# neu-vi/Superpoints_Registration

Hardware: AMD Instinct MI355X
Metric: point-cloud pairs/sec (16 384 pts/cloud) (higher is better)
Workload: dtype f32 (matrix products: range-scaled split-f16x2 MFMA, f32 accumulate; attention weights below 2^-5 of their row sum carried in one f16 plane); 1 GPU; synthetic 16384-pt pairs, full KPConv backbone + superpoint attn + Sinkhorn-SVD pose (3dmatch config, BASELINE configs[1]); streams_per_gpu=1, points_per_cloud=16384, generator=box, point_order=reference, upsample_indices=True, cross_step_overlap=True, streams_inside_a_forward=3: main path, pyramid searches, ResNet shortcut branches

## Files before the change

superpoints_registration_amd/csrc/kpconv.hip:

```cpp
#include "lds_dma.h"
#include "spr_common.h"
#include "split_mma.h"

namespace spr {
namespace {

constexpr int kKP = 15;

__global__ __launch_bounds__(256) void k_rowflag(const float* __restrict__ x, const float* __restrict__ s_xyz,
                                                 int ns, int cin, unsigned char* __restrict__ flag,
                                                 float4* __restrict__ sxf, int* __restrict__ tile_ctr) {
  const int wid = (blockIdx.x * blockDim.x + threadIdx.x) >> 6;
  const int lane = threadIdx.x & 63;
  const int c4 = cin >> 2;
  if (blockIdx.x == 0 && threadIdx.x == 0) {
    sxf[ns] = make_float4(-1.0e17f, -1.0e17f, -1.0e17f, __int_as_float(0));
    tile_ctr[0] = 0;
  }
  if ((cin & 3) == 0 && c4 <= 64 && (c4 & (c4 - 1)) == 0) {
    constexpr int kRfSteps = 4;
    const int rpl = 64 / c4;
    const int sub = lane / c4, chunk = lane % c4;
    const int row0 = wid * rpl * kRfSteps + sub;
    float4 v[kRfSteps];
// ... 428 lines not shown
  const int qv = lane & 15, g = lane >> 4;
  const int q0 = blockIdx.x * 64 + wave * 16;
  const int q = q0 + qv;
  float mx = 0.f;
  if (q0 < nq) {
    float b[4];
    stem_load_group(S, q0, nq, qv, g, b);
    const int cloud = find_segment(cu, nb, min(q, nq - 1));
    for (int o0 = 0; o0 < cout; o0 += 16) {
      f32x4 acc = {0.f, 0.f, 0.f, 0.f};
#pragma unroll
      for (int s = 0; s < 4; ++s) {
        const float av = 4 * s + g < n_kp ? W[(size_t)(4 * s + g) * cout + o0 + qv] : 0.f;
        acc = __builtin_amdgcn_mfma_f32_16x16x4f32(av, b[s], acc, 0, 0, 0);
      }
      if (q < nq) {
        const float4 m = *reinterpret_cast<const float4*>(mean + (size_t)cloud * cout + o0 + 4 * g);
        const float4 r = *reinterpret_cast<const float4*>(rstd + (size_t)cloud * cout + o0 + 4 * g);
        float4 w;
        w.x = (acc[0] - m.x) * r.x;
        w.y = (acc[1] - m.y) * r.y;
        w.z = (acc[2] - m.z) * r.z;
        w.w = (acc[3] - m.w) * r.w;
        w.x = w.x >= 0.f ? w.x : w.x * slope;
        w.y = w.y >= 0.f ? w.y : w.y * slope;
        w.z = w.z >= 0.f ? w.z : w.z * slope;
        w.w = w.w >= 0.f ? w.w : w.w * slope;
        *reinterpret_cast<float4*>(out + (size_t)q * cout + o0 + 4 * g) = w;
        mx = fmaxf(mx, fmaxf(fmaxf(fabsf(w.x), fabsf(w.y)), fmaxf(fabsf(w.z), fabsf(w.w))));
      }
    }
  }
  if (out_range != nullptr) publish_range(mx, out_range, nslots);
}

__global__ __launch_bounds__(256) void k_w_prep(const float* __restrict__ W, int cin, int cout, int cc,
                                                const float* __restrict__ w_parts, int n_wparts,
                                                _Float16* __restrict__ Wh, _Float16* __restrict__ Wl) {
  __shared__ float sh[17];
  const float sb = pow2f(pow2_exp_for(block_absmax(w_parts, sh, n_wparts)));
  const int total = kKP * cin * cout;
  const int i = blockIdx.x * blockDim.x + threadIdx.x;
  if (i >= total) return;
  const int KS = kKP * cc / 32, NT = cout / 16;
  const int e = i & 7, lane = (i >> 3) & 63;
  int r = i >> 9;
  const int ks = r % KS;
  r /= KS;
  const int nt = r % NT, chunk = r / NT;
  const int p16 = lane & 15, j4 = lane >> 4;
  const int kk = 32 * ks + 8 * j4 + e;
  const int p = kk / cc, c = chunk * cc + kk % cc;
  const float w = W[((size_t)p * cin + c) * cout + 16 * nt + p16] * sb;
  const _Float16 h = (_Float16)w;
  Wh[i] = h;
  Wl[i] = (_Float16)(w - (float)h);
}

#define KP_TILE_COUNTS(W) W(0) W(2) W(4) W(6) W(8) W(12) W(16)
SPR_DEFINE_WAIT_VM_ANY(wait_vm_tile, KP_TILE_COUNTS)

template <int N> struct VecF;
template <> struct VecF<2> { typedef f32x2 type; };
template <> struct VecF<4> { typedef f32x4 type; };
template <int N> struct VecH;
template <> struct VecH<2> { typedef f16x2 type; };
template <> struct VecH<4> { typedef f16x4 type; };

template <int NTC>
struct KpItem {
  int idx[4];
  float4 sp[4];
  float b[4][NTC];
  float qx, qy, qz;
};

template <int CC, int TQ, int NTW, int NW, int SK, int P1W>
__global__ __launch_bounds__(64 * P1W) void k_kpconv_mfma(
    const float* __restrict__ q_xyz, int nq, const float* __restrict__ s_xyz, int ns,
    const int* __restrict__ nbr, int nbr_stride, int kmax, int rows_sorted,
    const float* __restrict__ x, int cin, const _Float16* __restrict__ Wh,
    const _Float16* __restrict__ Wl, int cout, const float* __restrict__ kpts, float inv_extent,
    const float4* __restrict__ sxf, const float* __restrict__ x_parts,
    const float* __restrict__ w_parts, int n_xparts, int n_wparts, float* __restrict__ out) {
  constexpr int NTC = CC / 16;
  constexpr int MT = TQ / 16;
  constexpr int KW = kKP * CC;
  constexpr int SH = KW + 16;
  constexpr int QPW = TQ / P1W;
  constexpr int NTHR = 64 * P1W;
  static_assert(P1W >= NW && TQ % P1W == 0, "phase-1 waves");
  extern __shared__ __align__(16) unsigned char lds_raw[];
  _Float16* wfh = (_Float16*)lds_raw;
  _Float16* wfl = wfh + TQ * SH;
  int* lcnt = (int*)(wfl + TQ * SH);
  int* lnit = lcnt + TQ;
  int* litem = lnit + P1W;
  const int nblk = (kmax + 15) >> 4;
  const int KP = nblk * 16;
  int* lidx = litem + P1W * QPW * nblk;

  const int tid = threadIdx.x;
  const int wave = tid >> 6, lane = tid & 63;
  const int p16 = lane & 15, j4 = lane >> 4;

  float kx = 0.f, ky = 0.f, kz = 0.f;
  if (p16 < kKP) {
    kx = kpts[3 * p16];
    ky = kpts[3 * p16 + 1];
    kz = kpts[3 * p16 + 2];
  }

  float sa, unscale;
  {
    float* shf = reinterpret_cast<float*>(lds_raw);
    const int ka = pow2_exp_for(block_absmax(x_parts, shf, n_xparts) * (float)kmax);
    const int kb = pow2_exp_for(block_absmax(w_parts, shf, n_wparts));
    __syncthreads();
    sa = pow2f(ka);
    unscale = pow2f(-ka - kb);
  }

  const int ntiles = (nq + TQ - 1) / TQ;
  for (int tile = blockIdx.x; tile < ntiles; tile += gridDim.x) {
  const int q0 = tile * TQ;

  for (int e = tid; e < TQ * KP; e += NTHR) {
    const int q = e / KP, k = e - q * KP;
    const int n = q0 + q;
    lidx[e] = (n < nq && k < kmax) ? nbr[(size_t)n * nbr_stride + k] : ns;
  }
  __syncthreads();
  {
    int n_it = 0;
    for (int qi = 0; qi < QPW; ++qi) {
      const int* row = lidx + (wave * QPW + qi) * KP;
      int nb = nblk;
      if (rows_sorted) {
        int v = 0;
        for (int k0 = 0; k0 < KP; k0 += 64) {
          const int k = k0 + lane;
          const bool ok = k < KP && row[min(k, KP - 1)] >= 0 && row[min(k, KP - 1)] < ns;
          v += __popcll(__ballot(ok));
        }
        nb = max(1, (v + 15) >> 4);
      }
      if (lane < nb) litem[wave * QPW * nblk + n_it + lane] = (qi << 8) | ((lane == nb - 1) ? 128 : 0) | lane;
      n_it += nb;
    }
    if (lane == 0) lnit[wave] = n_it;
  }
  __syncthreads();
  const int n_items = lnit[wave];
  const int* my_items = litem + wave * QPW * nblk;

  constexpr int NG = (SK == 1) ? NW / MT : NW / SK;
  constexpr int MTW = (SK == 1) ? 1 : MT;
  const int mt = (SK == 1) ? wave % MT : 0;
  const int ng = (SK == 1) ? wave / MT : wave % NG;
  const int kh = (SK == 1) ? 0 : wave / NG;
  f32x4 acc2[MTW][NTW];
#pragma unroll
  for (int m = 0; m < MTW; ++m)
#pragma unroll
    for (int t = 0; t < NTW; ++t) acc2[m][t] = (f32x4){0.f, 0.f, 0.f, 0.f};

  for (int c0 = 0; c0 < cin; c0 += CC) {
    f32x4 acc1[NTC];
#pragma unroll
    for (int t = 0; t < NTC; ++t) acc1[t] = (f32x4){0.f, 0.f, 0.f, 0.f};
    int cnt = 0;

    auto issue = [&](int it, KpItem<NTC>& I) {
      const int code = my_items[min(it, n_items - 1)];
      const int qi = code >> 8, b = code & 127;
      const int n = min(q0 + wave * QPW + qi, nq - 1);
      const int* row = lidx + (wave * QPW + qi) * KP + b * 16 + j4;
      I.qx = q_xyz[3 * (size_t)n];
      I.qy = q_xyz[3 * (size_t)n + 1];
      I.qz = q_xyz[3 * (size_t)n + 2];
#pragma unroll
      for (int s = 0; s < 4; ++s) {
        const int id_ = row[4 * s];
        I.idx[s] = id_;
        const bool ok = id_ >= 0 && id_ < ns;
        const size_t id = ok ? (size_t)id_ : 0;
        I.sp[s] = sxf[id];
        typedef typename VecF<NTC>::type vec_t;
        const vec_t xv = *reinterpret_cast<const vec_t*>(x + id * cin + c0 + NTC * p16);
#pragma unroll
        for (int t = 0; t < NTC; ++t) I.b[s][t] = xv[t];
      }
    };
    auto compute = [&](int it, const KpItem<NTC>& I) {
      if (it >= n_items) return;
      const int code = my_items[it];
#pragma unroll
      for (int s = 0; s < 4; ++s) {
        const bool ok = I.idx[s] >= 0 && I.idx[s] < ns;
        const float dx = (I.sp[s].x - I.qx) - kx, dy = (I.sp[s].y - I.qy) - ky,
                    dz = (I.sp[s].z - I.qz) - kz;
        float w = fmaxf(0.f, 1.f - __builtin_amdgcn_sqrtf(dx * dx + dy * dy + dz * dz) * inv_extent);
        if (!ok || p16 >= kKP) w = 0.f;
        cnt += (ok && c0 == 0 && p16 == 0) ? __float_as_int(I.sp[s].w) : 0;
#pragma unroll
        for (int t = 0; t < NTC; ++t) {
          acc1[t] = __builtin_amdgcn_mfma_f32_16x16x4f32(w, I.b[s][t], acc1[t], 0, 0, 0);
        }
      }
      if (code & 128) {
        const int ql = wave * QPW + (code >> 8);
#pragma unroll
        for (int r = 0; r < 4; ++r) {
          const int p = acc_row16(r, j4);
          typedef typename VecH<NTC>::type hv_t;
          hv_t hh, ll;
          if constexpr (NTC == 2) {
            unsigned int hu, lu;
            split_pk_s(acc1[0][r], acc1[1][r], sa, hu, lu);
            hh = __builtin_bit_cast(hv_t, hu);
            ll = __builtin_bit_cast(hv_t, lu);
          } else {
            static_assert(NTC == 4, "NTC is 2 or 4");
            unsigned int h0, l0, h1, l1;
            split_pk_s(acc1[0][r], acc1[1][r], sa, h0, l0);
            split_pk_s(acc1[2][r], acc1[3][r], sa, h1, l1);
            hh = __builtin_bit_cast(hv_t, (u32x2){h0, h1});
            ll = __builtin_bit_cast(hv_t, (u32x2){l0, l1});
          }
          if (p < kKP) {
            *reinterpret_cast<hv_t*>(wfh + ql * SH + p * CC + NTC * p16) = hh;
            *reinterpret_cast<hv_t*>(wfl + ql * SH + p * CC + NTC * p16) = ll;
          }
        }
#pragma unroll
        for (int t = 0; t < NTC; ++t) acc1[t] = (f32x4){0.f, 0.f, 0.f, 0.f};
        if (c0 == 0) {
          int c = cnt;
          c += __shfl_xor(c, 16, 64);
          c += __shfl_xor(c, 32, 64);
          if (lane == 0) lcnt[ql] = c;
        }
        cnt = 0;
      }
    };

    {
      KpItem<NTC> A, B;
      issue(0, A);
      for (int it = 0; it < n_items; it += 2) {
        issue(it + 1, B);
        compute(it, A);
        issue(it + 2, A);
        compute(it + 1, B);
      }
    }
    __syncthreads();
    if (wave < NW) {
      constexpr int NBATCH = KW / 32 / SK;
      const int ks0 = kh * NBATCH;
      constexpr int LPB = 2 * NTW;
      constexpr int D = (NTW <= 2) ? 5 : 3;
      static_assert(NBATCH % D == 0 && NBATCH >= 2 * D && (D - 1) * LPB <= 16, "ring shape");
      const _Float16* ah_row = wfh + (mt * 16 + p16) * SH + 8 * j4;
      const _Float16* al_row = wfl + (mt * 16 + p16) * SH + 8 * j4;
      constexpr int KS = KW / 32;
      const size_t wofs = ((size_t)(c0 / CC) * (cout / 16) + ng * NTW) * KS * 512 + lane * 8;
      f16x8 bh[D][NTW], bl[D][NTW];
      auto load_step = [&](int ks, f16x8 (&dh)[NTW], f16x8 (&dl)[NTW]) {
        const size_t gk = wofs + (size_t)(ks0 + ks) * 512;
#pragma unroll
        for (int t = 0; t < NTW; ++t) {
          const _Float16* ph = Wh + gk + (size_t)t * KS * 512;
          const _Float16* pl = Wl + gk + (size_t)t * KS * 512;
          asm volatile("global_load_dwordx4 %0, %1, off" : "=v"(dh[t]) : "v"(ph));
          asm volatile("global_load_dwordx4 %0, %1, off" : "=v"(dl[t]) : "v"(pl));
        }
      };
      auto mma_step = [&](int ks, const f16x8 (&sh)[NTW], const f16x8 (&sl)[NTW]) {
#pragma unroll
        for (int m = 0; m < MTW; ++m) {
          const f16x8 ah = *reinterpret_cast<const f16x8*>(ah_row + m * 16 * SH + 32 * (ks0 + ks));
          const f16x8 al = *reinterpret_cast<const f16x8*>(al_row + m * 16 * SH + 32 * (ks0 + ks));
#pragma unroll
          for (int t = 0; t < NTW; ++t) {
            acc2[m][t] = mma3_16(ah, al, sh[t], sl[t], acc2[m][t]);
          }
        }
      };
      wait_vm<0>();
#pragma unroll
      for (int d = 0; d < D; ++d) load_step(d, bh[d], bl[d]);
      for (int b0 = 0; b0 < NBATCH - D; b0 += D) {
#pragma unroll
        for (int d = 0; d < D; ++d) {
          wait_vm_tile((D - 1) * LPB);
          __builtin_amdgcn_sched_barrier(0);
          mma_step(b0 + d, bh[d], bl[d]);
          __builtin_amdgcn_sched_barrier(0);
          load_step(b0 + d + D, bh[d], bl[d]);
        }
      }
#pragma unroll
      for (int d = 0; d < D; ++d) {
        wait_vm_tile((D - 1 - d) * LPB);
        __builtin_amdgcn_sched_barrier(0);
        mma_step(NBATCH - D + d, bh[d], bl[d]);
      }
    }
    __syncthreads();
  }
  const bool writer = (SK == 1) ? (wave < NW) : (wave < NW && kh == 0);
  if (SK == 2) {
    float* red = reinterpret_cast<float*>(lds_raw);
    if (wave < NW && kh == 1) {
#pragma unroll
      for (int m = 0; m < MTW; ++m)
#pragma unroll
        for (int t = 0; t < NTW; ++t)
#pragma unroll
          for (int r = 0; r < 4; ++r)
            red[(((ng * MTW + m) * NTW + t) * 4 + r) * 64 + lane] = acc2[m][t][r];
    }
    __syncthreads();
    if (writer) {
#pragma unroll
      for (int m = 0; m < MTW; ++m)
#pragma unroll
        for (int t = 0; t < NTW; ++t)
#pragma unroll
          for (int r = 0; r < 4; ++r)
            acc2[m][t][r] += red[(((ng * MTW + m) * NTW + t) * 4 + r) * 64 + lane];
    }
  }
  if (writer) {
#pragma unroll
    for (int m = 0; m < MTW; ++m)
#pragma unroll
      for (int r = 0; r < 4; ++r) {
        const int ql = (mt + m) * 16 + 4 * j4 + r;
        const int n = q0 + ql;
        if (n < nq) {
          const float inv = unscale / (float)max(lcnt[ql], 1);
#pragma unroll
          for (int t = 0; t < NTW; ++t)
            out[(size_t)n * cout + (ng * NTW + t) * 16 + p16] = acc2[m][t][r] * inv;
        }
      }
  }
  __syncthreads();
  }
}

static inline size_t mfma_lds_bytes(int cc, int tq, int p1w, int kmax) {
  const int sh = kKP * cc + 16, qpw = tq / p1w, nblk = (kmax + 15) / 16;
  return 2 * sizeof(_Float16) * (size_t)tq * sh + sizeof(int) * (tq + p1w) + sizeof(int) * (size_t)p1w * qpw * nblk +
         sizeof(int) * (size_t)tq * nblk * 16;
}
constexpr size_t kMfmaLdsMax = 160 * 1024;
constexpr int kTile64TQ = 32, kTile32TQ = 64, kTileWaves = 8;

template <int CC, int TQ, int NTW, int NW, int SK, int P1W = NW>
int launch_mfma(const float* q_xyz, int nq, const float* s_xyz, int ns, const int* nbr,
                int nbr_stride, int kmax, int rows_sorted, const float* x, int cin,
                const _Float16* Wh, const _Float16* Wl, int cout, const float* kpts,
                float inv_extent, const float4* sxf, const float* x_parts, const float* w_parts, int n_xparts,
                int n_wparts, float* out, hipStream_t stream) {
  const size_t lds = mfma_lds_bytes(CC, TQ, P1W, kmax);
  auto kern = k_kpconv_mfma<CC, TQ, NTW, NW, SK, P1W>;
  ProfScope prof(stream, cin * 100000 + cout, nq);
  SPR_REQUIRE(lds <= kMfmaLdsMax, "kpconv: neighbour rows too wide for the LDS tile (kmax=%d)", kmax);
  if (lds > 64 * 1024)
    if (int rc = ensure_dyn_lds((const void*)kern, 160 * 1024)) return rc;
  const int n_cu = device_cu_count();
  const int per_cu = (int)((160 * 1024) / lds) > 0 ? (int)((160 * 1024) / lds) : 1;
  const int ntiles = cdiv(nq, TQ);
  const int grid = ntiles < n_cu * per_cu ? ntiles : n_cu * per_cu;
  hipLaunchKernelGGL(kern, dim3(grid), dim3(64 * P1W), lds, stream, q_xyz, nq, s_xyz, ns,
                     nbr, nbr_stride, kmax, rows_sorted, x, cin, Wh, Wl, cout, kpts, inv_extent,
                     sxf, x_parts, w_parts, n_xparts, n_wparts, out);
  SPR_LAUNCH_CHECK();
  return 0;
}


constexpr int kRingTQ = 16;

__global__ __launch_bounds__(256) void k_kp_tiles(const int* __restrict__ nbr, int nq, int ns, int nbr_stride,
                                                  int kmax, int rows_sorted, const int* __restrict__ order,
                                                  int ntiles, int4* __restrict__ desc, int* __restrict__ pad_word) {
  const int tile = (blockIdx.x * blockDim.x + threadIdx.x) >> 6;
  const int lane = threadIdx.x & 63;
  if (blockIdx.x == 0 && threadIdx.x == 0) pad_word[0] = ns;
  if (tile >= ntiles) return;
  int my_q = -1, my_c = 0;
  for (int r = 0; r < kRingTQ; ++r) {
    const int pos = tile * kRingTQ + r;
    int q = -1, c = 0;
    if (pos < nq) {
      q = order ? order[pos] : pos;
      if (rows_sorted) {
        int v = 0;
        for (int k0 = 0; k0 < kmax; k0 += 64) {
          const int k = k0 + lane;
          const int id = k < kmax ? nbr[(size_t)q * nbr_stride + k] : ns;
          v += __popcll(__ballot(id >= 0 && id < ns));
        }
        c = max(1, (v + 7) >> 3);
      } else {
        c = (kmax + 7) >> 3;
      }
    }
    if (lane == r) { my_q = q; my_c = c; }
  }
  int rank = 0;
  for (int j = 0; j < kRingTQ; ++j) {
    const int cj = __shfl(my_c, j, 64);
    rank += (cj > my_c || (cj == my_c && j < lane)) ? 1 : 0;
  }
  if (lane < kRingTQ) {
    int* d = reinterpret_cast<int*>(desc + (size_t)tile * 8);
    const int w = rank < 8 ? rank : 15 - rank, second = rank < 8 ? 0 : 1;
    d[w * 4 + second] = my_q;
    d[w * 4 + 2 + second] = my_c;
  }
}

#define KP_RING_COUNTS(W)                                                                                      \
  W(0) W(1) W(2) W(3) W(4) W(5) W(6) W(7) W(8) W(9) W(10) W(11) W(12) W(13) W(14) W(15) W(16) W(17) W(18) W(19) \
  W(20) W(21) W(22) W(23) W(24) W(25) W(26) W(27) W(28)
SPR_DEFINE_WAIT_VM_ANY(wait_vm_ring, KP_RING_COUNTS)

template <int CC, int COUT, int NS>
struct RingShape {
  static constexpr int NTC = CC / 16;
  static constexpr int KW = kKP * CC;
  static constexpr int SH = KW + 16;
  static constexpr int KS = KW / 32;
  static constexpr int NG = COUT / 16;
  static constexpr int SPLIT = 8 / NG;
  static constexpr int KSW = (KS + SPLIT - 1) / SPLIT;
  static constexpr int RB = CC * 4;
  static constexpr int LPR = RB / 16;
  static constexpr int RPP = 64 / LPR;
  static constexpr int PPI = 8 / RPP;
  static constexpr int DPI = PPI + 1;
  static constexpr int SLOT = 8 * RB + 128;
  static constexpr int WF_BYTES = 2 * kRingTQ * SH * 2;
  static constexpr int RED_BYTES = NG * (SPLIT - 1) * 4 * 64 * 4;
  static constexpr int RING_BYTES = 8 * NS * SLOT;
  static constexpr int SMALL_BYTES = 2 * kRingTQ * 4 * 2 + 16;
  static constexpr int MINW = (CC == 32 && COUT == 32) ? 4 : 2;
  static_assert(NG * SPLIT == 8 && NS >= 3, "shape");
  static __host__ __device__ size_t lds_bytes(int idxw) {
    return (size_t)WF_BYTES + RED_BYTES + RING_BYTES + SMALL_BYTES + (size_t)8 * 2 * 2 * idxw * 4;
  }
};

#ifdef SPR_KP_RING_PROF
constexpr int kTraceN = 160;
__device__ unsigned long long g_kp_trace[8 * kTraceN];
#define KP_STAMP(id)                                                                            \
  do {                                                                                          \
// ... 276 lines not shown
        const int ks = min(ks0 + k, KS - 1);
        const f16x8 ah = *reinterpret_cast<const f16x8*>(ah_row + 32 * ks);
        const f16x8 al = *reinterpret_cast<const f16x8*>(al_row + 32 * ks);
        acc2 = mma3_16(ah, al, bh[k], bl[k], acc2);
      }
    }
    if (sp > 0) {
#pragma unroll
      for (int r = 0; r < 4; ++r) red[((ng * (SPLIT - 1) + sp - 1) * 4 + r) * 64 + lane] = acc2[r];
    }
    KP_STAMP(6);
    asm volatile("s_waitcnt lgkmcnt(0)" ::: "memory");
    __builtin_amdgcn_s_barrier();
    KP_STAMP(7);
    if (sp == 0) {
#pragma unroll
      for (int s2 = 1; s2 < SPLIT; ++s2)
#pragma unroll
        for (int r = 0; r < 4; ++r) acc2[r] += red[((ng * (SPLIT - 1) + s2 - 1) * 4 + r) * 64 + lane];
#pragma unroll
      for (int r = 0; r < 4; ++r) {
        const int ql = acc_row16(r, j4);
        pend_n[r] = lqid[par * kRingTQ + ql];
        const float inv = unscale / (float)max(lcnt[par * kRingTQ + ql], 1);
        pend_v[r] = acc2[r] * inv;
      }
    }
    KP_STAMP(8);
    d_cur = d_nxt;
    d_nxt = d_nn;
    tile = tile_nxt;
    tile_nxt = tile_nn;
    tile_nn = __builtin_amdgcn_readfirstlane(ltile[1 + par]);
  }
  if (sp == 0) flush_pending();
  wait_vm<0>();
#ifdef SPR_KP_RING_PROF
  if (blockIdx.x == 0) {
    asm volatile("s_waitcnt lgkmcnt(0)" ::: "memory");
    for (int k = lane; k < kTraceN; k += 64) g_kp_trace[wave * kTraceN + k] = k < trace_n ? trace_lds[wave * kTraceN + k] : 0ull;
  }
#endif
}

template <int CC, int COUT, int NS>
int launch_ring(const float* q_xyz, int nq, int ns, const int* nbr, int nbr_stride, int kmax, const float* x,
                const _Float16* Wh, const _Float16* Wl, const float* kpts, float inv_extent, const float4* sxf,
                const int4* desc, const int* pad_word, const float* x_parts, const float* w_parts, int n_xparts,
                int n_wparts, int* tile_ctr, float* out, hipStream_t stream) {
  typedef RingShape<CC, COUT, NS> S;
  const int idxw = kmax <= 64 ? 64 : 128;
#ifdef SPR_KP_RING_PROF
  const size_t lds = S::lds_bytes(idxw) + 8 * kTraceN * 8;
#else
  const size_t lds = S::lds_bytes(idxw);
#endif
  auto kern = k_kpconv_ring<CC, COUT, NS>;
  ProfScope prof(stream, CC * 100000 + COUT, nq);
  if (lds > 64 * 1024)
    if (int rc = ensure_dyn_lds((const void*)kern, 160 * 1024)) return rc;
  const int ntiles = cdiv(nq, kRingTQ);
  const int n_cu = device_cu_count();
  int per_cu = (int)((160 * 1024) / lds);
  per_cu = per_cu < 1 ? 1 : (per_cu > S::MINW / 2 ? S::MINW / 2 : per_cu);
  const int grid = ntiles < n_cu * per_cu ? ntiles : n_cu * per_cu;
  hipLaunchKernelGGL(kern, dim3(grid), dim3(512), lds, stream, q_xyz, ns, nbr, nbr_stride, kmax, x, Wh, Wl, kpts,
                     inv_extent, sxf, desc, ntiles, pad_word, idxw, x_parts, w_parts, n_xparts, n_wparts, tile_ctr, out);
  SPR_LAUNCH_CHECK();
  return 0;
}

}

void launch_rowflag(const float* x, const float* s_xyz, int ns, int cin, unsigned char* flag, float4* sxf,
                    int* tile_ctr, hipStream_t stream) {
  const int c4 = cin >> 2;
  const bool wide = (cin & 3) == 0 && c4 <= 64 && (c4 & (c4 - 1)) == 0;
  const long waves = wide ? cdiv(ns, (64 / c4) * 4) : (long)ns;
  hipLaunchKernelGGL(k_rowflag, dim3(cdiv(waves * 64, 256)), dim3(256), 0, stream, x, s_xyz, ns, cin, flag, sxf, tile_ctr);
}
}

using namespace spr;

#ifdef SPR_KP_RING_PROF
extern "C" int spr_debug_kp_trace(unsigned long long* out, int n) {
  if (hipDeviceSynchronize() != hipSuccess) return 1;
  if (hipMemcpyFromSymbol(out, HIP_SYMBOL(g_kp_trace), sizeof(unsigned long long) * n) != hipSuccess) return 1;
  return 0;
}
#endif

struct KpPlan {
  int4* desc;
  int* pad_word;
};
static KpPlan plan_view(Workspace& w, int nq) {
  KpPlan p;
  p.desc = w.take<int4>((size_t)cdiv(nq > 0 ? nq : 1, kRingTQ) * 8);
  p.pad_word = w.take<int>(64);
  return p;
}
struct KpWPlanes {
  _Float16 *hi, *lo;
};
static KpWPlanes wplanes_view(Workspace& w, int cin, int cout) {
  const size_t n = (size_t)32 * (size_t)(cin > 0 ? cin : 0) * (size_t)(cout > 0 ? cout : 0);
  KpWPlanes p;
  p.hi = w.take<_Float16>(n);
  p.lo = w.take<_Float16>(n);
  return p;
}
struct KpWs {
  unsigned char* flag;
  float4* sxf;
  KpWPlanes wplanes;
  float *x_parts, *w_parts;
  KpPlan plan;
  int* tile_ctr;
  float4* few_rec;
};
static inline bool few_cin(int cin) { return cin >= 2 && cin <= 8; }
static KpWs kpconv_layout(Workspace& w, int nq, int ns, int cin, int cout) {
  const size_t n = (size_t)(ns > 0 ? ns : 1);
  KpWs l;
  l.flag = w.take<unsigned char>(n);
  l.sxf = w.take<float4>(n + 1);
  l.wplanes = wplanes_view(w, cin, cout);
  l.x_parts = w.take<float>(kAmaxParts);
  l.w_parts = w.take<float>(kAmaxParts);
  l.plan = plan_view(w, nq);
  l.tile_ctr = w.take<int>(64);
  l.few_rec = w.take<float4>(cin >= 2 ? n * (cin <= 4 ? 2 : 3) : 0);
  return l;
}
static inline int w_chunk(int cin) { return cin % 64 == 0 ? 64 : 32; }
static inline bool ring_shape(int cin, int cout) {
  return (cin == 32 || cin == 64) && cin * cout <= 4096 && cout % 32 == 0 && 8 % (cout / 16) == 0;
}

extern "C" size_t spr_kpconv_plan_bytes(int nq) {
  return measure(plan_view, nq);
}

static int launch_plan(const int* nbr, int nq, int ns, int nbr_stride, int kmax, int rows_sorted, const int* order,
                       const KpPlan& p, hipStream_t stream) {
  const int ntiles = cdiv(nq, kRingTQ);
  hipLaunchKernelGGL(k_kp_tiles, dim3(cdiv((long)ntiles * 64, 256)), dim3(256), 0, stream, nbr, nq, ns, nbr_stride,
                     kmax, rows_sorted, order, ntiles, p.desc, p.pad_word);
  SPR_LAUNCH_CHECK();
  return 0;
}

extern "C" int spr_kpconv_plan(const int* nbr, int nq, int ns, int nbr_stride, int kmax, int rows_sorted,
                               const int* order, void* plan, size_t plan_bytes, void* stream_) {
  hipStream_t stream = (hipStream_t)stream_;
  SPR_REQUIRE(nq > 0 && ns > 0 && kmax >= 1 && kmax <= nbr_stride, "kpconv plan: bad sizes");
  Workspace w(plan, plan_bytes);
  const KpPlan p = plan_view(w, nq);
  SPR_REQUIRE(plan != nullptr && w.ok(), "kpconv plan: buffer too small");
  return launch_plan(nbr, nq, ns, nbr_stride, kmax, rows_sorted, order, p, stream);
}

extern "C" size_t spr_kpconv_wplanes_bytes(int cin, int cout) {
  return measure(wplanes_view, cin, cout);
}
// ... 91 lines not shown
                              const float* x, int cin, const float* weights, int cout,
                              const float* kernel_points, int n_kp, float kp_extent,
                              float* out, int impl, const float* x_range, int x_range_n, const float* w_range,
                              int w_range_n, const void* plan, const void* wplanes, void* ws, size_t ws_bytes,
                              void* stream_) {
  hipStream_t stream = (hipStream_t)stream_;
  SPR_REQUIRE((x_range == nullptr || x_range_n >= 1) && (w_range == nullptr || w_range_n >= 1),
              "kpconv: a range needs a count");
  SPR_REQUIRE(nq > 0 && ns > 0, "kpconv: empty input");
  SPR_REQUIRE(kmax >= 1 && kmax <= nbr_stride, "kpconv: bad kmax=%d stride=%d", kmax, nbr_stride);
  SPR_REQUIRE(cin >= 1 && cout >= 1 && n_kp >= 1 && n_kp <= 32, "kpconv: bad dims");
  SPR_REQUIRE(kp_extent > 0.f, "kpconv: KP_extent must be > 0");
  Workspace w(ws, ws_bytes);
  const auto [flag, sxf, own_wplanes, x_parts, w_parts, own_plan, tile_ctr, few_rec] = kpconv_layout(w, nq, ns, cin, cout);
  SPR_REQUIRE(ws != nullptr && w.ok(), "kpconv: workspace too small");
  SPR_REQUIRE(wplanes == nullptr || w_range != nullptr, "kpconv: prepared weight planes come with the range they were scaled by");
  Workspace given_w(const_cast<void*>(wplanes), SIZE_MAX), given_p(const_cast<void*>(plan), SIZE_MAX);
  const auto [wh, wl] = wplanes != nullptr ? wplanes_view(given_w, cin, cout) : own_wplanes;
  const float inv_extent = 1.0f / kp_extent;

  if (cin == 1 && (impl == 0 || impl == 2) && n_kp <= 16) {
    hipLaunchKernelGGL(k_records_cin1, dim3(cdiv(ns, 256)), dim3(256), 0, stream, x, s_xyz, ns, sxf);
    ProfScope prof(stream, cin * 100000 + cout, nq);
    hipLaunchKernelGGL(k_kpconv_cin1, dim3(cdiv(nq, 64)), dim3(256), 0, stream, q_xyz, nq, s_xyz, ns, nbr,
                       nbr_stride, kmax, rows_sorted, sxf, weights, cout, kernel_points, n_kp, inv_extent, out);
    SPR_LAUNCH_CHECK();
    return 0;
  }

  if ((impl == 0 || impl == 2) && spr_kpconv_few_supported(cin, cout, n_kp)) {
    switch (cin) {
#define SPR_FEW_CASE(C)                                                                                              \
  case C: {                                                                                                          \
    hipLaunchKernelGGL(k_records_few<C>, dim3(cdiv(ns, 256)), dim3(256), 0, stream, x, s_xyz, ns, few_rec);          \
    ProfScope prof(stream, cin * 100000 + cout, nq);                                                                 \
    hipLaunchKernelGGL(k_kpconv_few<C>, dim3(cdiv(nq, 64)), dim3(256), 0, stream, q_xyz, nq, ns, nbr, nbr_stride,    \
                       kmax, rows_sorted, few_rec, weights, cout, kernel_points, n_kp, inv_extent, out);             \
  } break;
      SPR_FEW_CASE(2) SPR_FEW_CASE(3) SPR_FEW_CASE(4) SPR_FEW_CASE(5) SPR_FEW_CASE(6) SPR_FEW_CASE(7) SPR_FEW_CASE(8)
#undef SPR_FEW_CASE
    }
    SPR_LAUNCH_CHECK();
    return 0;
  }

  launch_rowflag(x, s_xyz, ns, cin, flag, sxf, tile_ctr, stream);
  SPR_LAUNCH_CHECK();

  const bool tile_fits = cin % 64 == 0 ? mfma_lds_bytes(64, kTile64TQ, kTileWaves, kmax) <= kMfmaLdsMax
                                       : mfma_lds_bytes(32, kTile32TQ, kTileWaves, kmax) <= kMfmaLdsMax;
  if ((impl == 0 || impl == 2) && n_kp == kKP && cin % 32 == 0 && cout % 32 == 0 && cout <= 256 && tile_fits) {
    const int ktot = n_kp * cin;
    const float* xp = x_range != nullptr ? x_range : x_parts;
    const float* wp = w_range != nullptr ? w_range : w_parts;
    const int n_xp = x_range != nullptr ? x_range_n : kAmaxParts, n_wp = w_range != nullptr ? w_range_n : kAmaxParts;
    if (x_range == nullptr && w_range == nullptr) {
      if (int rc = launch_absmax2(x, ns, cin, cin, x_parts, weights, ktot, cout, cout, w_parts, stream)) return rc;
    } else if (x_range == nullptr) {
      if (int rc = launch_absmax(x, ns, cin, cin, x_parts, stream)) return rc;
    } else if (w_range == nullptr) {
      if (int rc = launch_absmax(weights, ktot, cout, cout, w_parts, stream)) return rc;
    }
    if (wplanes == nullptr)
      hipLaunchKernelGGL(k_w_prep, dim3(cdiv((long)ktot * cout, 256)), dim3(256), 0, stream, weights, cin, cout,
                         w_chunk(cin), wp, n_wp, wh, wl);
    const bool ring_ok = impl == 0 && ring_shape(cin, cout) && kmax <= 128 && (size_t)ns * cin * 4 < (1ull << 32) &&
                         (size_t)nq * nbr_stride * 4 < (1ull << 32);
    if (ring_ok) {
      if (plan == nullptr)
        if (int rc = launch_plan(nbr, nq, ns, nbr_stride, kmax, rows_sorted, nullptr, own_plan, stream)) return rc;
      const auto [desc, pad_word] = plan != nullptr ? plan_view(given_p, nq) : own_plan;
#define SPR_RING_ARGS                                                                                       \
  q_xyz, nq, ns, nbr, nbr_stride, kmax, x, wh, wl, kernel_points, inv_extent, sxf, desc, pad_word, xp, wp, \
      n_xp, n_wp, tile_ctr, out, stream
      if (cin == 64 && cout == 64) return launch_ring<64, 64, 4>(SPR_RING_ARGS);
      if (cin == 64 && cout == 32) return launch_ring<64, 32, 4>(SPR_RING_ARGS);
      if (cin == 32 && cout == 32) return launch_ring<32, 32, 3>(SPR_RING_ARGS);
      if (cin == 32 && cout == 64) return launch_ring<32, 64, 8>(SPR_RING_ARGS);
      if (cin == 32 && cout == 128) return launch_ring<32, 128, 8>(SPR_RING_ARGS);
#undef SPR_RING_ARGS
    }
#define SPR_KP_ARGS                                                                         \
  q_xyz, nq, s_xyz, ns, nbr, nbr_stride, kmax, rows_sorted, x, cin, wh, wl, cout,           \
      kernel_points, inv_extent, sxf, xp, wp, n_xp, n_wp, out, stream
    if (cin % 64 == 0) {
      if (cout == 64) return launch_mfma<64, kTile64TQ, 1, kTileWaves, 2>(SPR_KP_ARGS);
      if (cout == 128) return launch_mfma<64, kTile64TQ, 2, kTileWaves, 2>(SPR_KP_ARGS);
      if (cout == 256) return launch_mfma<64, kTile64TQ, 4, kTileWaves, 2>(SPR_KP_ARGS);
    } else {
      if (cout == 32) return launch_mfma<32, kTile32TQ, 1, kTileWaves, 1>(SPR_KP_ARGS);
      if (cout == 64) return launch_mfma<32, kTile32TQ, 2, kTileWaves, 1>(SPR_KP_ARGS);
      if (cout == 128) return launch_mfma<32, kTile32TQ, 4, kTileWaves, 1>(SPR_KP_ARGS);
    }
#undef SPR_KP_ARGS
  }
  const long total = (long)nq * cout;
  hipLaunchKernelGGL(k_kpconv_simple, dim3(cdiv(total, 256)), dim3(256), 0, stream, q_xyz, nq,
                     s_xyz, ns, nbr, nbr_stride, kmax, x, cin, weights, cout, kernel_points, n_kp,
                     inv_extent, flag, out);
  SPR_LAUNCH_CHECK();
  return 0;
}
```

superpoints_registration_amd/ops.py:

```python
import ctypes
import math
import threading
from typing import Optional, Sequence, Tuple

import numpy as np
import torch

from . import _lib

ACT_NONE, ACT_RELU, ACT_SIGMOID = 0, 1, 2
ORDER_REFERENCE, ORDER_CANONICAL = 0, 1
SELECT_NEAREST, SELECT_INDEX = 0, 1


def _stream(t: torch.Tensor):
    return ctypes.c_void_p(torch.cuda.current_stream(t.device).cuda_stream)


def _ptr(t: Optional[torch.Tensor]):
    return None if t is None else ctypes.c_void_p(t.data_ptr())


def _dev(t: torch.Tensor, name: str, dtype=None) -> torch.Tensor:
    if not isinstance(t, torch.Tensor) or not t.is_cuda:
# ... 515 lines not shown


def kpconv(q_pts, s_pts, nbr, x, weights, kernel_points, kp_extent: float, rows_sorted: bool = False,
           impl: int = 0) -> torch.Tensor:
    if _wants_grad(x, weights):
        from .autograd import KPConvFn
        return KPConvFn.apply(_dev(q_pts, "q_pts", torch.float32), _dev(s_pts, "s_pts", torch.float32), nbr,
                              _dev(x, "x", torch.float32), weights, kernel_points, float(kp_extent),
                              bool(rows_sorted), int(impl))
    return kpconv_raw(q_pts, s_pts, nbr, x, weights, kernel_points, kp_extent, rows_sorted, impl)


def kpconv_raw(q_pts, s_pts, nbr, x, weights, kernel_points, kp_extent: float, rows_sorted: bool = False,
               impl: int = 0, order: Optional[torch.Tensor] = None) -> torch.Tensor:
    q_pts = _dev(q_pts, "q_pts", torch.float32)
    s_pts = _dev(s_pts, "s_pts", torch.float32)
    x = _dev(x, "x", torch.float32)
    weights = _dev(weights, "weights", torch.float32)
    kernel_points = _dev(kernel_points, "kernel_points", torch.float32)
    if not nbr.is_cuda:
        raise RuntimeError("neighb_inds must be on the device")
    if nbr.dtype != torch.int32:
        nbr = nbr.to(torch.int32)
    stride = nbr.stride(0) if nbr.stride(1) == 1 and nbr.shape[1] > 0 else None
    if stride is None:
        nbr = nbr.contiguous()
        stride = nbr.shape[1]
    nq, ns, kmax = q_pts.shape[0], s_pts.shape[0], nbr.shape[1]
    n_kp, cin, cout = weights.shape
    assert x.shape == (ns, cin), (x.shape, ns, cin)
    L = _lib.lib()
    ws = _workspace(L.spr_kpconv_workspace_bytes(nq, ns, cin, cout), x.device)
    out = torch.empty((nq, cout), dtype=torch.float32, device=x.device)
    xr, xr_n = _get_range(x)
    wr, wr_n = _static_range(weights)
    plan = wplanes = None
    if impl == 0 and n_kp == 15 and cin % 32 == 0 and cout % 32 == 0 and cout <= 256:
        if cin in (32, 64) and cin * cout <= 4096 and kmax <= 128:
            plan = _kpconv_plan(nbr, nq, ns, int(stride), kmax, bool(rows_sorted), order)
        if wr is not None:
            wplanes = _kpconv_wplanes(weights, wr, wr_n)
    _lib.check(L.spr_kpconv_fwd(_ptr(q_pts), nq, _ptr(s_pts), ns, _ptr(nbr), int(stride), kmax,
                                int(bool(rows_sorted)), _ptr(x), cin, _ptr(weights), cout,
                                _ptr(kernel_points), n_kp, float(kp_extent), _ptr(out), int(impl),
                                _ptr(xr), int(xr_n), _ptr(wr), int(wr_n), _ptr(plan), _ptr(wplanes),
                                _ptr(ws), ws.numel(), _stream(x)), "spr_kpconv_fwd")
    return out


def _kpconv_plan(nbr: torch.Tensor, nq: int, ns: int, stride: int, kmax: int, rows_sorted: bool,
                 order: Optional[torch.Tensor] = None) -> torch.Tensor:
    if order is not None:
        order = _dev(order, "order", torch.int32)
        assert order.shape == (nq,)

    def build():
        L = _lib.lib()
        nbytes = L.spr_kpconv_plan_bytes(nq)
        plan = torch.empty((nbytes,), dtype=torch.uint8, device=nbr.device)
        _lib.check(L.spr_kpconv_plan(_ptr(nbr), nq, ns, stride, kmax, int(rows_sorted), _ptr(order), _ptr(plan),
                                     nbytes, _stream(nbr)), "spr_kpconv_plan")
        return plan, plan
    return _derived(nbr, '_spr_kp_plan', (nq, ns, stride, kmax, rows_sorted, None if order is None else _ident(order)),
                    build)


def kpconv_plan_prefetch(nbr: torch.Tensor, ns: int, rows_sorted: bool = True) -> None:
    if nbr is None or not nbr.is_cuda or nbr.dtype != torch.int32 or nbr.dim() != 2 or nbr.shape[1] < 1:
        return
    if nbr.stride(1) != 1 or nbr.shape[1] > 128 or nbr.shape[0] < 1:
        return
    _kpconv_plan(nbr, nbr.shape[0], int(ns), int(nbr.stride(0)), nbr.shape[1], bool(rows_sorted))


def _kpconv_wplanes(weights: torch.Tensor, wr: torch.Tensor, wr_n: int) -> torch.Tensor:
    def build():
        L = _lib.lib()
        n_kp, cin, cout = weights.shape
        nbytes = L.spr_kpconv_wplanes_bytes(cin, cout)
        planes = torch.empty((nbytes,), dtype=torch.uint8, device=weights.device)
        _lib.check(L.spr_kpconv_prep_weights(_ptr(weights), n_kp, cin, cout, _ptr(wr), int(wr_n), _ptr(planes),
                                             nbytes, _stream(weights)), "spr_kpconv_prep_weights")
        return planes, planes
    return _derived(weights, '_spr_kp_wplanes', wr.data_ptr(), build)


def instnorm(x, cu, eps: float = 1e-5, norm: bool = True, add=None, slope: float = 1.0,
             out=None, max_len: Optional[int] = None) -> torch.Tensor:
    if _wants_grad(x, add):
        from .autograd import InstNormFn
        return InstNormFn.apply(_dev(x, "x", torch.float32), _dev(cu, "cu", torch.int32), float(eps), bool(norm),
                                None if add is None else _dev(add, "add", torch.float32), float(slope), max_len)
    return instnorm_raw(x, cu, eps, norm, add, slope, out, max_len)


def instnorm_raw(x, cu, eps: float = 1e-5, norm: bool = True, add=None, slope: float = 1.0,
                 out=None, max_len: Optional[int] = None) -> torch.Tensor:
    x = _dev(x, "x", torch.float32)
    cu = _dev(cu, "cu", torch.int32)
    n, c = x.shape
    nb = cu.numel() - 1
    if add is not None:
        add = _dev(add, "add", torch.float32)
        assert add.shape == x.shape
    if out is None:
        out = torch.empty_like(x)
    L = _lib.lib()
    max_len = n if max_len is None else max(1, min(int(max_len), n))
    ws = _workspace(L.spr_instnorm_workspace_bytes(max_len, nb, c), x.device)
    cnt = _STREAM_SLOTS
    rng = _zero_slots(cnt, x.device)
    _lib.check(L.spr_instnorm(_ptr(x), _ptr(cu), n, nb, max_len, c, float(eps), int(bool(norm)), _ptr(add),
                              float(slope), _ptr(out), _ptr(rng), cnt, _ptr(ws), ws.numel(), _stream(x)),
               "spr_instnorm")
    _set_range(out, rng, cnt)
    return out


def block_tail_tile_rows(ka: int, kb: int, n_out: int) -> int:
    if _modes["gemm"] != 1:
        return 0
    return int(_lib.lib().spr_block_tail_tile_rows(int(ka), int(kb), int(n_out)))


def _tail_tiles(cu: torch.Tensor, n: int, tr: int) -> torch.Tensor:
    def build():
        L = _lib.lib()
        t = torch.empty((L.spr_block_tail_tiles_len(n, cu.numel() - 1, tr),), dtype=torch.int32, device=cu.device)
        _lib.check(L.spr_block_tail_tiles(_ptr(cu), n, cu.numel() - 1, tr, _ptr(t), _stream(cu)), "spr_block_tail_tiles")
        return t, t
    return _derived(cu, f'_spr_tail_tiles_{tr}', (n, tr), build)


def instnorm_stats(x, cu, eps: float = 1e-5, max_len: Optional[int] = None):
    x = _dev(x, "x", torch.float32)
    cu = _dev(cu, "cu", torch.int32)
    n, c = x.shape
    nb = cu.numel() - 1
    L = _lib.lib()
    max_len = n if max_len is None else max(1, min(int(max_len), n))
    ws = _workspace(L.spr_instnorm_workspace_bytes(max_len, nb, c), x.device)
    st = torch.empty((2, nb, c), dtype=torch.float32, device=x.device)
    _lib.check(L.spr_instnorm_stats(_ptr(x), _ptr(cu), n, nb, max_len, c, float(eps), _ptr(st[0]), _ptr(st[1]),
                                    _ptr(ws), ws.numel(), _stream(x)), "spr_instnorm_stats")
    return st[0], st[1]


_NORM_BOUNDS = {}


def _norm_bound(max_len: int, device) -> torch.Tensor:
    key = (int(max_len), str(device))
    t = _NORM_BOUNDS.get(key)
    if t is None:
        t = torch.full((1,), float(max(1, int(max_len))) ** 0.5, dtype=torch.float32, device=device)
        _NORM_BOUNDS[key] = t
    return t


def block_tail(xa, wa, cu, xb=None, wb=None, add=None, eps: float = 1e-5, slope: float = 0.1,
               xa_stats=None, xa_slope: float = 0.1, xa_max_len: Optional[int] = None) -> torch.Tensor:
    xa = _dev(xa, "xa", torch.float32)
    wa = _dev(wa, "wa", torch.float32)
    cu = _dev(cu, "cu", torch.int32)
    n, ka = xa.shape
    n_out = wa.shape[0]
    assert wa.shape[1] == ka
# ... 929 lines not shown
```

Baseline: 1285 pairs/s.

## Use atomic work-stealing tile scheduler and SGPR-based weight loads in KPConv MFMA kernel

Swaps the static grid-stride tile loop for dynamic tile claiming through a global atomic counter, which k_rowflag resets. Each block prefetches its next tile index while it works on the current one, so blocks with uneven neighbour counts balance their load. The weight-plane loads now use a scalar base plus a 32-bit VGPR offset instead of 64-bit per-lane pointers, and the MMA ring loop is fully unrolled so step counts need not divide by the ring depth. The ops.py change adds the weight shape to the plane cache key.

```diff
diff --git a/superpoints_registration_amd/csrc/kpconv.hip b/superpoints_registration_amd/csrc/kpconv.hip
--- a/superpoints_registration_amd/csrc/kpconv.hip
+++ b/superpoints_registration_amd/csrc/kpconv.hip
@@ -534,7 +534,8 @@
     const float* __restrict__ x, int cin, const _Float16* __restrict__ Wh,
     const _Float16* __restrict__ Wl, int cout, const float* __restrict__ kpts, float inv_extent,
     const float4* __restrict__ sxf, const float* __restrict__ x_parts,
-    const float* __restrict__ w_parts, int n_xparts, int n_wparts, float* __restrict__ out) {
+    const float* __restrict__ w_parts, int n_xparts, int n_wparts, int* __restrict__ tile_ctr,
+    float* __restrict__ out) {
   constexpr int NTC = CC / 16;
   constexpr int MT = TQ / 16;
   constexpr int KW = kKP * CC;
@@ -547,7 +548,8 @@
   _Float16* wfl = wfh + TQ * SH;
   int* lcnt = (int*)(wfl + TQ * SH);
   int* lnit = lcnt + TQ;
-  int* litem = lnit + P1W;
+  int* ltile = lnit + P1W;
+  int* litem = ltile + 2;
   const int nblk = (kmax + 15) >> 4;
   const int KP = nblk * 16;
   int* lidx = litem + P1W * QPW * nblk;
@@ -565,6 +567,7 @@
 
   float sa, unscale;
   {
+    if (tid == 0) ltile[0] = __hip_atomic_fetch_add(tile_ctr, 1, __ATOMIC_RELAXED, __HIP_MEMORY_SCOPE_AGENT);
     float* shf = reinterpret_cast<float*>(lds_raw);
     const int ka = pow2_exp_for(block_absmax(x_parts, shf, n_xparts) * (float)kmax);
     const int kb = pow2_exp_for(block_absmax(w_parts, shf, n_wparts));
@@ -574,8 +577,11 @@
   }
 
   const int ntiles = (nq + TQ - 1) / TQ;
-  for (int tile = blockIdx.x; tile < ntiles; tile += gridDim.x) {
+  int tile = __builtin_amdgcn_readfirstlane(ltile[0]);
+  while (tile < ntiles) {
   const int q0 = tile * TQ;
+  int drawn = ntiles;
+  if (tid == 0) drawn = __hip_atomic_fetch_add(tile_ctr, 1, __ATOMIC_RELAXED, __HIP_MEMORY_SCOPE_AGENT);
 
   for (int e = tid; e < TQ * KP; e += NTHR) {
     const int q = e / KP, k = e - q * KP;
@@ -709,55 +715,47 @@
     }
     __syncthreads();
     if (wave < NW) {
-      constexpr int NBATCH = KW / 32 / SK;
-      const int ks0 = kh * NBATCH;
+      constexpr int KS = KW / 32;
+      constexpr int NB = KS / SK;
       constexpr int LPB = 2 * NTW;
       constexpr int D = (NTW <= 2) ? 5 : 3;
-      static_assert(NBATCH % D == 0 && NBATCH >= 2 * D && (D - 1) * LPB <= 16, "ring shape");
+      static_assert(KS % SK == 0 && NB > D && (D - 1) * LPB <= 16, "ring shape");
       const _Float16* ah_row = wfh + (mt * 16 + p16) * SH + 8 * j4;
       const _Float16* al_row = wfl + (mt * 16 + p16) * SH + 8 * j4;
-      constexpr int KS = KW / 32;
-      const size_t wofs = ((size_t)(c0 / CC) * (cout / 16) + ng * NTW) * KS * 512 + lane * 8;
-      f16x8 bh[D][NTW], bl[D][NTW];
+      const unsigned wofs =
+          ((((unsigned)(c0 / CC) * (cout / 16) + ng * NTW) * KS + kh * NB) * 512 + lane * 8) * (unsigned)sizeof(_Float16);
       auto load_step = [&](int ks, f16x8 (&dh)[NTW], f16x8 (&dl)[NTW]) {
-        const size_t gk = wofs + (size_t)(ks0 + ks) * 512;
 #pragma unroll
         for (int t = 0; t < NTW; ++t) {
-          const _Float16* ph = Wh + gk + (size_t)t * KS * 512;
-          const _Float16* pl = Wl + gk + (size_t)t * KS * 512;
-          asm volatile("global_load_dwordx4 %0, %1, off" : "=v"(dh[t]) : "v"(ph));
-          asm volatile("global_load_dwordx4 %0, %1, off" : "=v"(dl[t]) : "v"(pl));
+          const unsigned off = wofs + (unsigned)(ks + t * KS) * 1024u;
+          asm volatile("global_load_dwordx4 %0, %1, %2" : "=v"(dh[t]) : "v"(off), "s"(Wh));
+          asm volatile("global_load_dwordx4 %0, %1, %2" : "=v"(dl[t]) : "v"(off), "s"(Wl));
         }
       };
       auto mma_step = [&](int ks, const f16x8 (&sh)[NTW], const f16x8 (&sl)[NTW]) {
 #pragma unroll
         for (int m = 0; m < MTW; ++m) {
-          const f16x8 ah = *reinterpret_cast<const f16x8*>(ah_row + m * 16 * SH + 32 * (ks0 + ks));
-          const f16x8 al = *reinterpret_cast<const f16x8*>(al_row + m * 16 * SH + 32 * (ks0 + ks));
+          const f16x8 ah = *reinterpret_cast<const f16x8*>(ah_row + m * 16 * SH + 32 * (kh * NB + ks));
+          const f16x8 al = *reinterpret_cast<const f16x8*>(al_row + m * 16 * SH + 32 * (kh * NB + ks));
 #pragma unroll
           for (int t = 0; t < NTW; ++t) {
             acc2[m][t] = mma3_16(ah, al, sh[t], sl[t], acc2[m][t]);
           }
         }
       };
+      f16x8 bh[D][NTW], bl[D][NTW];
       wait_vm<0>();
 #pragma unroll
       for (int d = 0; d < D; ++d) load_step(d, bh[d], bl[d]);
-      for (int b0 = 0; b0 < NBATCH - D; b0 += D) {
-#pragma unroll
-        for (int d = 0; d < D; ++d) {
-          wait_vm_tile((D - 1) * LPB);
+#pragma unroll
+      for (int k = 0; k < NB; ++k) {
+        wait_vm_tile((D - 1 < NB - 1 - k ? D - 1 : NB - 1 - k) * LPB);
+        __builtin_amdgcn_sched_barrier(0);
+        mma_step(k, bh[k % D], bl[k % D]);
+        if (k + D < NB) {
           __builtin_amdgcn_sched_barrier(0);
-          mma_step(b0 + d, bh[d], bl[d]);
-          __builtin_amdgcn_sched_barrier(0);
-          load_step(b0 + d + D, bh[d], bl[d]);
+          load_step(k + D, bh[k % D], bl[k % D]);
         }
-      }
-#pragma unroll
-      for (int d = 0; d < D; ++d) {
-        wait_vm_tile((D - 1 - d) * LPB);
-        __builtin_amdgcn_sched_barrier(0);
-        mma_step(NBATCH - D + d, bh[d], bl[d]);
       }
     }
     __syncthreads();
@@ -800,13 +798,15 @@
         }
       }
   }
+  if (tid == 0) ltile[1] = drawn;
   __syncthreads();
+  tile = __builtin_amdgcn_readfirstlane(ltile[1]);
   }
 }
 
 static inline size_t mfma_lds_bytes(int cc, int tq, int p1w, int kmax) {
   const int sh = kKP * cc + 16, qpw = tq / p1w, nblk = (kmax + 15) / 16;
-  return 2 * sizeof(_Float16) * (size_t)tq * sh + sizeof(int) * (tq + p1w) + sizeof(int) * (size_t)p1w * qpw * nblk +
+  return 2 * sizeof(_Float16) * (size_t)tq * sh + sizeof(int) * (tq + p1w + 2) + sizeof(int) * (size_t)p1w * qpw * nblk +
          sizeof(int) * (size_t)tq * nblk * 16;
 }
 constexpr size_t kMfmaLdsMax = 160 * 1024;
@@ -817,7 +817,7 @@
                 int nbr_stride, int kmax, int rows_sorted, const float* x, int cin,
                 const _Float16* Wh, const _Float16* Wl, int cout, const float* kpts,
                 float inv_extent, const float4* sxf, const float* x_parts, const float* w_parts, int n_xparts,
-                int n_wparts, float* out, hipStream_t stream) {
+                int n_wparts, int* tile_ctr, float* out, hipStream_t stream) {
   const size_t lds = mfma_lds_bytes(CC, TQ, P1W, kmax);
   auto kern = k_kpconv_mfma<CC, TQ, NTW, NW, SK, P1W>;
   ProfScope prof(stream, cin * 100000 + cout, nq);
@@ -830,7 +830,7 @@
   const int grid = ntiles < n_cu * per_cu ? ntiles : n_cu * per_cu;
   hipLaunchKernelGGL(kern, dim3(grid), dim3(64 * P1W), lds, stream, q_xyz, nq, s_xyz, ns,
                      nbr, nbr_stride, kmax, rows_sorted, x, cin, Wh, Wl, cout, kpts, inv_extent,
-                     sxf, x_parts, w_parts, n_xparts, n_wparts, out);
+                     sxf, x_parts, w_parts, n_xparts, n_wparts, tile_ctr, out);
   SPR_LAUNCH_CHECK();
   return 0;
 }
@@ -1273,6 +1273,7 @@
 }
 
 using namespace spr;
+
 
 #ifdef SPR_KP_RING_PROF
 extern "C" int spr_debug_kp_trace(unsigned long long* out, int n) {
@@ -1530,7 +1531,7 @@
     }
 #define SPR_KP_ARGS                                                                         \
   q_xyz, nq, s_xyz, ns, nbr, nbr_stride, kmax, rows_sorted, x, cin, wh, wl, cout,           \
-      kernel_points, inv_extent, sxf, xp, wp, n_xp, n_wp, out, stream
+      kernel_points, inv_extent, sxf, xp, wp, n_xp, n_wp, tile_ctr, out, stream
     if (cin % 64 == 0) {
       if (cout == 64) return launch_mfma<64, kTile64TQ, 1, kTileWaves, 2>(SPR_KP_ARGS);
       if (cout == 128) return launch_mfma<64, kTile64TQ, 2, kTileWaves, 2>(SPR_KP_ARGS);
diff --git a/superpoints_registration_amd/ops.py b/superpoints_registration_amd/ops.py
--- a/superpoints_registration_amd/ops.py
+++ b/superpoints_registration_amd/ops.py
@@ -621,7 +621,7 @@
         _lib.check(L.spr_kpconv_prep_weights(_ptr(weights), n_kp, cin, cout, _ptr(wr), int(wr_n), _ptr(planes),
                                              nbytes, _stream(weights)), "spr_kpconv_prep_weights")
         return planes, planes
-    return _derived(weights, '_spr_kp_wplanes', wr.data_ptr(), build)
+    return _derived(weights, '_spr_kp_wplanes', (wr.data_ptr(), tuple(weights.shape)), build)
 
 
 def instnorm(x, cu, eps: float = 1e-5, norm: bool = True, add=None, slope: float = 1.0,
```

Result: no change. 1283 pairs/s (-0.2%).
